# sile/libflate

Measured on AMD Instinct MI355X. Metric: gzip encode+decode throughput on 256 MiB synthetic text per GPU (uncompressed bytes through the round trip), higher is better.
Workload: dtype u8; 1 GPU; cfg2: gzip::Encoder (DefaultLz77Encoder, default options, mtime=0) + gzip::Decoder on TEXT(268435456 B) per GPU, write schedule S8K (8192-byte writes); bytes_per_gpu=268435456, schedule=S8K, compressed_bytes=129579521, parallelism=1 rank

## Files before the change

### libflate_amd/csrc/lfx_decode.cpp

```cpp
#include "../../include/lfx.h"

#include <hip/hip_runtime.h>

#include <algorithm>
#include <cstddef>
#include <cstdio>
#include <cstdlib>
#include <cstring>
#include <mutex>
#include <string>
#include <vector>

#include "lfx_decode_int.h"
#include "lfx_container.h"
#include "lfx_index.h"
#include "lfx_bgzf.h"
#include "lfx_dict.h"

static_assert(offsetof(lfx::DecStream, out_off) == 16 && sizeof(lfx::DecStream) % 8 == 0, "checksum_ranges stride");
static_assert(offsetof(lfx::InflateResult, out_len) == 8 && sizeof(lfx::InflateResult) % 8 == 0, "checksum_ranges stride");
#include "lfx_device.h"
#include "lfx_abi_guard.h"

using namespace lfx;

namespace {

int size_member(Ctx *c, const uint8_t *d_in, uint64_t n, uint64_t off0, MemberResult &mr);

int verify_trailer(Ctx *c, int format, const uint8_t *d_in, uint64_t tpos, uint64_t need, const uint8_t *d_out, const MemberResult &mr,
                   DecodeOutcome &oc) {
    hipStream_t st = c->stream;
    uint8_t t[8];
    EncodeResult er{};
    if (mr.ck_done) {
        er.crc32 = mr.crc32; er.adler32 = mr.adler32;
        memcpy(t, mr.trailer, need);
    } else {
        const uint64_t nspans = ck_nspans(mr.out_len);
        int rc;
        if ((rc = c->d_ck.reserve(12 * nspans))) return rc;
        uint32_t *ck = (uint32_t *)c->d_ck.p;
        LAUNCH_TRY(launch_checksum(st, d_out, mr.out_len, ck, ck + nspans, ck + 2 * nspans, (EncodeResult *)c->d_res.p,
                                   format == LFX_GZIP ? 1 : format == LFX_ZLIB ? 2 : 3));
        HIP_TRY(hipMemcpyAsync(c->h_res, c->d_res.p, sizeof(EncodeResult), hipMemcpyDeviceToHost, st));
        HIP_TRY(hipMemcpyAsync(t, d_in + tpos, need, hipMemcpyDeviceToHost, st));
        HIP_TRY(hipStreamSynchronize(st));
        c->phase("checksum");
        er = *(EncodeResult *)c->h_res;
    }
    if (const int bad = check_trailer(format, t, er.crc32, er.adler32, oc.msg)) oc.status = bad;
    return LFX_OK;
}

int member_loop(Ctx *c, int format, uint32_t flags, const uint8_t *d_in, uint64_t n, uint8_t *d_out, uint64_t cap, bool sizes_only,
                DecodeOutcome &oc, uint64_t base, uint64_t out_at, bool one_member, std::vector<lfx_member> *members,
                const lfx_dict *dict = nullptr) {
    (void)hipSetDevice(c->device);
    hipStream_t st = c->stream;
    bool first = base == 0;
    oc.consumed = base;
    oc.out_len = oc.delivered_len = out_at;
    int rc;
    if (!sizes_only && (rc = c->d_res.reserve(256))) return rc;
    if ((rc = c->d_small.reserve(70000))) return rc;
    for (;;) {
        uint64_t off0 = 0;
        uint64_t dict_hist = dict && format == LFX_DEFLATE ? dict->usable : 0;
        if (format != LFX_DEFLATE) {
            DecStream ds{base, n - base, 0, 0};
            DecHeader dh{};
            c->pin_reset();
            HIP_TRY(c->small_up(c->d_small.p, &ds, sizeof ds, st));
            if (dict)
                LAUNCH_TRY(launch_container_dict(st, 1, d_in, (const DecStream *)c->d_small.p,
                                                 (DecHeader *)((uint8_t *)c->d_small.p + 256), dict->id));
            else
            LAUNCH_TRY(launch_container(st, format, 1, d_in, (const DecStream *)c->d_small.p,
                                        (DecHeader *)((uint8_t *)c->d_small.p + 256)));
            HIP_TRY(c->small_down(&dh, (uint8_t *)c->d_small.p + 256, sizeof dh, st));
            HIP_TRY(c->small_sync(st));
            if (dh.status != 0) {
                if (!first && dh.status == 2) {
                    oc.consumed = n;
                    break;
                }
                oc.status = map_status(dh.status);
                oc.header_failed = first;
                oc.msg = format_error(dh.err, dh.a0, dh.a1);
                oc.consumed = base + dh.deflate_off;
                oc.out_len = oc.delivered_len = out_at;
                return LFX_OK;
            }
            off0 = dh.deflate_off;
            if (dict && (dh.flags & HDR_DICT)) dict_hist = dict->usable;
        }
        if (c->idx && !sizes_only) {
            c->idx->bit_base = base * 8;
            c->idx->out_base = out_at;
            c->idx->cand.push_back(IdxCand{(base + off0) * 8, (base + off0) * 8, out_at, IDX_BTYPE_READ});
        }
        MemberResult mr;
        if (sizes_only) rc = size_member(c, d_in + base, n - base, off0, mr);
        else {
            mr.ck_mode = ck_mode_of(format);
            mr.trailer_len = trailer_len(format);
            rc = inflate_member(c, d_in + base, n - base, off0, d_out + out_at, cap - out_at, mr, ~0ull, ~0ull, false, dict_hist,
                                dict_hist ? dict->d_win : nullptr);
        }
        if (rc) return rc;
        oc.out_len = out_at + mr.out_len;
        oc.delivered_len = out_at + mr.blk_out_start;
        oc.consumed = base + mr.end_byte;
        if (mr.status != LFX_OK) { oc.status = mr.status; oc.msg = mr.msg; return LFX_OK; }
        if (format != LFX_DEFLATE) {
            const uint64_t need = trailer_len(format);
            const uint64_t tpos = base + mr.end_byte;
            if (n - tpos < need) {
                oc.status = LFX_E_UNEXPECTED_EOF;
                oc.msg = "failed to fill whole buffer";
                oc.consumed = n;
                return LFX_OK;
            }
            oc.consumed = tpos + need;
            if (!sizes_only) {
                if ((rc = verify_trailer(c, format, d_in, tpos, need, d_out + out_at, mr, oc))) return rc;
                if (oc.status != LFX_OK) return LFX_OK;
            }
        }
        if (members) members->push_back(lfx_member{base, oc.consumed - base, out_at, mr.out_len});
        out_at = oc.out_len;
        if (one_member) { oc.more = true; break; }
        if (!(format == LFX_GZIP && (flags & LFX_DEC_MULTI))) break;
        base = oc.consumed;
        first = false;
    }
    oc.out_len = oc.delivered_len = out_at;
    return LFX_OK;
}

int decode_stream(Ctx *c, int format, uint32_t flags, const uint8_t *d_in, uint64_t n, uint8_t *d_out,
                  uint64_t cap, DecodeOutcome &oc, uint64_t base = 0, uint64_t out_at = 0, bool one_member = false,
                  std::vector<lfx_member> *members = nullptr, const lfx_dict *dict = nullptr) {
    return member_loop(c, format, flags, d_in, n, d_out, cap, false, oc, base, out_at, one_member, members, dict);
}

int parse_headers(Ctx *c, int format, const uint8_t *d_in, const std::vector<DecStream> &streams, std::vector<DecHeader> &hdrs,
                  size_t extra_bytes = 0, DecStream **d_streams = nullptr, DecHeader **d_hdrs = nullptr, const lfx_dict *dict = nullptr) {
    hipStream_t st = c->stream;
    const uint32_t count = (uint32_t)streams.size();
    const size_t sz_streams = sizeof(DecStream) * count, sz_hdr = sizeof(DecHeader) * count;
    int rc;
    if ((rc = c->d_dec_blocks.reserve(sz_streams + sz_hdr + extra_bytes))) return rc;
    DecStream *ds = (DecStream *)c->d_dec_blocks.p;
    DecHeader *dh = (DecHeader *)((uint8_t *)c->d_dec_blocks.p + sz_streams);
    HIP_TRY(hipMemcpyAsync(ds, streams.data(), sz_streams, hipMemcpyHostToDevice, st));
    if (dict && format == LFX_ZLIB) LAUNCH_TRY(launch_container_dict(st, count, d_in, ds, dh, dict->id));
    else LAUNCH_TRY(launch_container(st, format, count, d_in, ds, dh));
    hdrs.assign(count, DecHeader{});
    if (format != LFX_DEFLATE) {
        HIP_TRY(hipMemcpyAsync(hdrs.data(), dh, sz_hdr, hipMemcpyDeviceToHost, st));
// ... 1499 lines not shown
```

### libflate_amd/csrc/lfx_decode.h

```cpp
#pragma once
#include <hip/hip_runtime.h>
#include <stdint.h>

#include "lfx_common.h"
#include "lfx_blk.h"

namespace lfx {

struct DecStream {
    uint64_t in_off, in_len;
    uint64_t out_off, out_cap;
};
enum : uint32_t { JOB_SINGLE_BLOCK = 1, JOB_COUNT_ONLY = 2 };
struct InflateJob {
    uint64_t in_off;
    uint64_t in_len;
    uint64_t start_bit;
    uint64_t out_off, out_cap;
    uint64_t hist_avail;
    uint64_t stop_bit;
    uint32_t flags;
    uint32_t dict_len;
};
struct InflateResult {
// ... 27 lines not shown
int launch_blk_walk_size(hipStream_t st, const uint8_t *in, uint64_t nbytes, const WalkJob *jobs, uint32_t njobs,
                         WalkResult *results, bool small_blocks);
size_t blk_tabs_bytes();
int launch_blk_scan(hipStream_t st, const uint8_t *in, uint64_t nbytes, const BlkJob *jobs, uint32_t njobs,
                    BlkInfo *infos, BlkLanes *lanes, void *tabs = nullptr,
                    bool small_blocks = false);
int launch_blk_scan_store(hipStream_t st, const uint8_t *in, uint64_t nbytes, const BlkJob *jobs, uint32_t njobs,
                          BlkInfo *infos, BlkLanes *lanes, void *tabs, uint32_t *temp, BlkLanesX *lanesx);
int launch_blk_place(hipStream_t st, const BlkEmit *jobs, uint32_t njobs, const BlkLanes *lanes, const BlkLanesX *lanesx,
                     const uint32_t *temp, uint32_t *codes, uint32_t *flags, BlkUnits *units, uint32_t unit_target,
                     uint32_t *job_flags, uint32_t free_shift);
int launch_blk_emit(hipStream_t st, const uint8_t *in, uint64_t nbytes, const BlkEmit *jobs, uint32_t njobs,
                    const BlkLanes *lanes, uint32_t *codes, uint32_t *flags, BlkUnits *units, uint32_t unit_target,
                    uint32_t *job_flags = nullptr,
                    const void *tabs = nullptr,
                    uint32_t free_shift = 17,
                    bool large_blocks = false,
                    bool small_blocks = false);
int launch_blk_materialize(hipStream_t st, const uint8_t *in, const BlkEmit *jobs, uint32_t njobs,
                           const BlkLanes *lanes, const BlkUnits *units, const uint32_t *codes, uint8_t *out,
                           uint64_t *dbg);
int launch_blk_materialize_dict(hipStream_t st, const uint8_t *in, const BlkEmit *jobs, uint32_t njobs, const BlkUnits *units,
                                const uint32_t *codes, uint8_t *out, const uint8_t *dict_end);

int launch_blk_materialize_sym(hipStream_t st, const uint8_t *in, const BlkEmit *jobs, uint32_t njobs,
                               const BlkUnits *units, const uint32_t *codes, uint16_t *sym,
                               bool few_units = false );
int launch_window_chain(hipStream_t st, const uint16_t *sym, const SymUnit *units, uint32_t nunits, uint8_t *windows,
                        const uint8_t *init_win = nullptr);
size_t window_prefix_scratch_bytes(uint32_t nunits);
int launch_window_prefix(hipStream_t st, const uint16_t *sym, const SymUnit *units, uint32_t nunits, void *scratch,
                         uint8_t *windows, const uint8_t *init_win = nullptr);
int launch_window_rank_map(hipStream_t st, const uint16_t *sym, const SymUnit *units, uint32_t nunits, void *scratch, uint16_t *out_map);
int launch_bytes_to_map(hipStream_t st, const uint8_t *out, uint64_t len, uint16_t *map);
int launch_window_ranks(hipStream_t st, const uint16_t *maps, uint32_t nranks, uint8_t *win);
int launch_sym_substitute(hipStream_t st, const uint16_t *sym, const SymUnit *units, uint32_t nunits,
                          const uint8_t *windows, uint8_t *out, uint64_t max_len, const uint8_t *init_win = nullptr);

int launch_container(hipStream_t st, int format, uint32_t count, const uint8_t *in,
                     const DecStream *streams, DecHeader *hdrs);
int launch_inflate(hipStream_t st, const uint8_t *in, uint8_t *out, const InflateJob *jobs,
                   InflateResult *results, uint32_t njobs);
int launch_container_dict(hipStream_t st, uint32_t count, const uint8_t *in, const DecStream *streams, DecHeader *hdrs,
                          uint32_t dict_id);
int launch_inflate_dict(hipStream_t st, const uint8_t *in, uint8_t *out, const InflateJob *jobs, InflateResult *results,
                        uint32_t njobs, const uint8_t *dict_end);
constexpr uint32_t FIND_SHARDS = 256;
constexpr uint32_t FIND_HDR_WORDS = 1024, FIND_HDR_FINAL = 320, FIND_HDR_DBG = 360, FIND_HDR_READ = 512 ;
constexpr uint32_t FIND2_GROUPS = 16, FIND_HDR_WORK = 512, FIND_HDR_WORK_STRIDE = 32;
inline uint32_t find_shard_cap(uint64_t comp_bytes) {
    const uint64_t want = comp_bytes / 4000;
    return (uint32_t)(want < 4096 ? 4096 : want > (1u << 23) ? (1u << 23) : want);
}
int launch_find_stage1(hipStream_t st, const uint8_t *in, uint64_t nbytes, uint64_t first_byte,
                       uint32_t *count, uint64_t *cand, uint32_t shard_cap, uint64_t final_from_bit, uint32_t n_cu);
int launch_find_stage2(hipStream_t st, const uint8_t *in, uint64_t nbytes, const uint64_t *cand,
                       uint32_t shard_cap, const uint32_t *count ,
                       uint32_t *work ,
                       uint32_t *final_count, uint64_t *final_list, uint32_t final_cap, uint32_t n_cu,
                       uint64_t *dbg = nullptr ,
                       int exp = 0 );
constexpr uint64_t MEMBER_TILE = 16384;
constexpr uint64_t MEMBER_SKIP = ~0ull;
inline uint64_t member_tiles(uint64_t n) { return (n + MEMBER_TILE - 1) / MEMBER_TILE; }
int launch_member_count(hipStream_t st, const uint8_t *in, uint64_t n, uint32_t *tile_count );
int launch_member_emit(hipStream_t st, const uint8_t *in, uint64_t n, const uint64_t *tile_pos ,
                       uint64_t *out, uint64_t cap);
int launch_verify_trailers(hipStream_t st, int format, uint32_t count, const uint8_t *in,
                           const DecStream *streams, const DecHeader *hdrs, InflateResult *results,
                           const uint32_t *crc, const uint32_t *adler, uint64_t *consumed);
}
```

### libflate_amd/csrc/lfx_decode_int.h

```cpp
#pragma once
#include <hip/hip_runtime.h>

#include <string>
#include <vector>

#include "../../include/lfx.h"
#include "lfx_container.h"
#include "lfx_verdict.h"
#include "lfx_ctx.h"
#include "lfx_decode.h"
#include "lfx_stages.h"
#include "lfx_try.h"

namespace lfx {

struct MemberResult {
    int status = LFX_OK;
    uint64_t out_len = 0;
    uint64_t blk_out_start = 0;
    uint64_t end_byte = 0;
    std::string msg;
    uint64_t end_bit = 0;
    bool final_seen = false;
    bool need_cap = false;
    int ck_mode = 0;
    uint32_t trailer_len = 0;
    bool ck_done = false;
    uint32_t crc32 = 0, adler32 = 1;
    uint8_t trailer[8] = {0, 0, 0, 0, 0, 0, 0, 0};
};

struct DecodeOutcome {
    int status = LFX_OK;
    uint64_t out_len = 0, delivered_len = 0, consumed = 0;
    bool header_failed = false;
    bool more = false;
    std::string msg;
};

int run_jobs(Ctx *c, const uint8_t *d_in, uint8_t *d_out, const std::vector<InflateJob> &jobs, std::vector<InflateResult> &res,
             const uint8_t *dict_end = nullptr);

struct HuffProbe { uint64_t in_off, in_len; InflateResult r; };
inline bool huff_verdict(const InflateResult &r) { return r.status == 1 && r.err == ERR_HUFF; }
int huff_consumed(Ctx *c, const uint8_t *d_in, const std::vector<HuffProbe> &probes, std::vector<uint64_t> &used);

int inflate_member(Ctx *c, const uint8_t *d_in, uint64_t n, uint64_t off0, uint8_t *d_out, uint64_t cap, MemberResult &mr,
                   uint64_t start_bit0 = ~0ull, uint64_t stop_bit = ~0ull, bool partial = false, uint64_t hist = 0,
                   const uint8_t *hist_win = nullptr);


struct FindBufs {
    uint32_t shard_cap = 0, final_cap = 0;
    uint32_t *d_count = nullptr;
    uint64_t *d_final = nullptr;
    uint64_t *d_cand = nullptr;
};
struct Found {
    std::vector<uint64_t> cand;
    bool overflow = false;
    uint32_t n1 = 0;
};
int find_launch(Ctx *c, const uint8_t *d_in, uint64_t n, uint64_t off0, uint64_t final_from, FindBufs &fb);
int find_collect(Ctx *c, const uint8_t *d_in, uint64_t n, const FindBufs &fb, Found &out);
inline uint64_t find_final_from(uint64_t n, uint64_t comp) {
    const uint64_t tail_bytes = std::max<uint64_t>(comp / 8, 8ull << 20);
    return comp > tail_bytes ? (n - tail_bytes) * 8 : 0;
}

bool plan_store(Ctx *c, BlkJob *bj, uint32_t nj);

int rescan_widen(Ctx *c, const uint8_t *d_in, uint64_t n, const std::vector<uint64_t> &starts, uint32_t nc,
                 std::vector<BlkInfo> &bi, std::vector<uint32_t> &slot, std::vector<uint8_t> &stored, bool scan_small);

struct EmitBufs {
    uint32_t *d_flags = nullptr;
    BlkEmit *d_emit = nullptr;
};
int emit_codes(Ctx *c, const uint8_t *d_in, uint64_t n, const std::vector<BlkEmit> &emit, uint64_t total_codes, uint32_t n_placed,
               uint32_t free_shift, bool scan_small, EmitBufs &eb);

int scan_round(Ctx *c, const uint8_t *d_in, uint64_t n, const std::vector<BlkJob> &bj, bool want_tabs, std::vector<BlkInfo> &bi,
               bool &small, bool stamp = false);
int emit_round(Ctx *c, const uint8_t *d_in, uint64_t n, const std::vector<BlkEmit> &emit, uint64_t total_codes, bool small,
               uint8_t *d_out, std::vector<uint32_t> &jf, bool stamp = false, const uint8_t *dict_end = nullptr);

}
```

### libflate_amd/csrc/lfx_decode_kernels.hip

```cpp
#include <hip/hip_runtime.h>
#include <stdint.h>

#include "lfx_common.h"
#include "lfx_decode.h"
#include "lfx_container.h"

namespace lfx {

__device__ __forceinline__ uint32_t ld1(gptr_u8 p) { return *p; }

__global__ void container_kernel(int format, uint32_t count, const uint8_t *__restrict__ in,
                                 const DecStream *__restrict__ streams, DecHeader *__restrict__ hdrs) {
    const uint32_t i = blockIdx.x * blockDim.x + threadIdx.x;
    if (i >= count) return;
    hdrs[i] = parse_container(format, in + streams[i].in_off, streams[i].in_len, nullptr);
}
__global__ void container_dict_kernel(uint32_t count, const uint8_t *__restrict__ in, const DecStream *__restrict__ streams,
                                      DecHeader *__restrict__ hdrs, uint32_t dict_id) {
    const uint32_t i = blockIdx.x * blockDim.x + threadIdx.x;
    if (i >= count) return;
    hdrs[i] = resolve_fdict(parse_container(1, in + streams[i].in_off, streams[i].in_len, nullptr), dict_id);
}

constexpr uint32_t WIN_BYTES = 2048;
// ... 173 lines not shown
#undef LFX_INFLATE_DICT

constexpr uint32_t FIND_DWORDS = 1024;
#ifndef LFX_FIND_FLUSH
#define LFX_FIND_FLUSH 4
#endif
constexpr uint32_t FIND_FLUSH = LFX_FIND_FLUSH;
constexpr uint32_t FIND_WL = 64 * FIND_FLUSH < 256 ? 256 : 64 * FIND_FLUSH;
constexpr uint32_t FIND_LIST = 4096;
struct FindLut { uint16_t v[4096]; };
constexpr FindLut make_find_lut() {
    FindLut t{};
    for (uint32_t i = 0; i < 4096; ++i) {
        uint32_t k = 0, u = 0;
        for (int f = 0; f < 4; ++f) { const uint32_t l = (i >> (3 * f)) & 7; if (l) { k += 128u >> l; u++; } }
        t.v[i] = (uint16_t)(k | (u << 12));
    }
    return t;
}
__device__ const FindLut g_find_lut = make_find_lut();

constexpr uint32_t FIND_CLASSES = 16, FIND_SUB = FIND_SHARDS / FIND_CLASSES;
static_assert(FIND_CLASSES * FIND_SUB == FIND_SHARDS, "lists");
struct FindCls { uint8_t v[512]; };
constexpr FindCls make_find_cls() {
    constexpr uint32_t th[15] = {432, 568, 652, 832, 944, 1076, 1420, 1604, 2008, 2710, 3016, 4978, 5184, 5664, 9820};
    FindCls t{};
    for (uint32_t i = 0; i < 512; ++i) {
        const uint32_t l16 = i & 7, l17 = (i >> 3) & 7, l18 = i >> 6;
        const uint32_t p16 = l16 ? 128u >> l16 : 0u, p17 = l17 ? 128u >> l17 : 0u, p18 = l18 ? 128u >> l18 : 0u;
        const uint32_t rest = p16 + p17 + p18 <= 128 ? 128 - p16 - p17 - p18 : 0;
        const uint32_t e2 = p18 * 149 + p17 * 13 + p16 * 9 + 2 * rest;
        uint32_t c = 0;
        for (uint32_t k = 0; k < 15; ++k) c += e2 >= th[k] ? 1u : 0u;
        t.v[i] = (uint8_t)c;
    }
    return t;
}
__device__ const FindCls g_find_cls = make_find_cls();

__device__ __forceinline__ uint32_t find_wave_inclusive_sum(uint32_t x) {
    x += (uint32_t)__builtin_amdgcn_update_dpp(0, (int)x, 0x111, 0xF, 0xF, true);
    x += (uint32_t)__builtin_amdgcn_update_dpp(0, (int)x, 0x112, 0xF, 0xF, true);
    x += (uint32_t)__builtin_amdgcn_update_dpp(0, (int)x, 0x114, 0xF, 0xF, true);
    x += (uint32_t)__builtin_amdgcn_update_dpp(0, (int)x, 0x118, 0xF, 0xF, true);
    x += (uint32_t)__builtin_amdgcn_update_dpp(0, (int)x, 0x142, 0xA, 0xF, false);
    x += (uint32_t)__builtin_amdgcn_update_dpp(0, (int)x, 0x143, 0xC, 0xF, false);
    return x;
}

__global__ __launch_bounds__(256) void find_blocks_stage1(const uint8_t *__restrict__ in, uint64_t nbytes,
                                                          uint64_t first_byte, uint32_t *__restrict__ count,
                                                          uint64_t *__restrict__ cand, uint32_t shard_cap,
                                                          uint64_t final_from_bit, uint32_t ntiles) {
    __shared__ __attribute__((aligned(16))) uint32_t sd[FIND_DWORDS + 4];
    __shared__ __attribute__((aligned(16))) uint16_t lut[4096];
    __shared__ uint16_t list[FIND_LIST];
    __shared__ uint64_t wl[FIND_WL];
    __shared__ uint32_t wn, s_wtot[4], ccnt[FIND_CLASSES], cbase[FIND_CLASSES];
    if (threadIdx.x == 0) wn = 0;
    if (threadIdx.x < FIND_CLASSES) ccnt[threadIdx.x] = 0;
    const uint32_t tid = threadIdx.x, lane = tid & 63, wave = tid >> 6;
    const uint64_t a = (uint64_t)in;
    gptr_u32 w = (gptr_u32)(a & ~3ull);
    const uint64_t shift = a & 3;
    const uint64_t wlast = (shift + nbytes + 3) / 4 - 1;
    const uint64_t stream_bits = nbytes * 8, lo_bit = first_byte * 8;
    const uint32_t sub = blockIdx.x % FIND_SUB;
    {
        const uint4 *gl = (const uint4 *)g_find_lut.v;
        const uint4 l0 = gl[tid], l1 = gl[tid + 256];
        ((uint4 *)lut)[tid] = l0;
        ((uint4 *)lut)[tid + 256] = l1;
    }
    uint32_t v[5];
    auto tile_w0 = [&](uint32_t tile) { return (first_byte + (uint64_t)tile * (4 * FIND_DWORDS) + shift) >> 2; };
    auto fetch = [&](uint32_t tile) {
        const uint64_t tw0 = tile_w0(tile);
#pragma unroll
        for (uint32_t k = 0; k < 5; ++k) { const uint64_t idx = tw0 + tid + 256 * k; v[k] = w[idx < wlast ? idx : wlast]; }
    };
    uint32_t done = 0;
    if (blockIdx.x < ntiles) fetch(blockIdx.x);
    for (uint32_t tile = blockIdx.x; tile < ntiles; tile += gridDim.x) {
        const uint64_t w0 = tile_w0(tile);
        __syncthreads();
#pragma unroll
        for (uint32_t k = 0; k < 5; ++k) { const uint32_t i = tid + 256 * k; if (i < FIND_DWORDS + 4) sd[i] = v[k]; }
        __syncthreads();
        if (tile + gridDim.x < ntiles) fetch(tile + gridDim.x);
        for (uint32_t t0 = 0; t0 < FIND_DWORDS; t0 += 256) {
            const uint32_t t = t0 + tid;
            const uint32_t d0 = sd[t], d1 = sd[t + 1];
            const uint64_t dword_bit0 = (4 * (w0 + t) - shift) * 8;
            const uint32_t allow_final = dword_bit0 + 32 > final_from_bit ? ~0u : 0u;
            const uint64_t lo = (uint64_t)d0 | (uint64_t)d1 << 32;
            uint32_t pm = (uint32_t)(~(lo >> 1) & (lo >> 2)) & (~d0 | allow_final);
            const uint32_t cnt = (uint32_t)__popc(pm);
            const uint32_t incl = find_wave_inclusive_sum(cnt);
            if (lane == 63) s_wtot[wave] = incl;
            __syncthreads();
            uint32_t pos = incl - cnt, total = 0;
#pragma unroll
            for (uint32_t j = 0; j < 4; ++j) { const uint32_t wj = s_wtot[j]; pos += j < wave ? wj : 0u; total += wj; }
            while (pm) {
                const uint32_t ph = (uint32_t)__builtin_ctz(pm);
                pm &= pm - 1;
                list[pos++] = (uint16_t)(t << 5 | ph);
            }
            __syncthreads();
            for (uint32_t i = tid; i < total; i += 256) {
                const uint32_t e = list[i], te = e >> 5, ph = e & 31;
                const uint32_t e0 = sd[te], e1 = sd[te + 1], e2 = sd[te + 2], e3 = sd[te + 3];
                const uint32_t x0 = __builtin_amdgcn_alignbit(e1, e0, ph), x1 = __builtin_amdgcn_alignbit(e2, e1, ph),
                               x2 = __builtin_amdgcn_alignbit(e3, e2, ph);
                const uint32_t hlit = (x0 >> 3) & 31, hdist = (x0 >> 8) & 31, hclen = (x0 >> 13) & 15;
                if (hlit > 29 || hdist > 29) continue;
                const uint32_t nb = 3 * (hclen + 4);
                uint32_t f0 = __builtin_amdgcn_alignbit(x1, x0, 17), f1 = __builtin_amdgcn_alignbit(x2, x1, 17);
                const uint32_t m0 = nb >= 32 ? ~0u : (1u << nb) - 1u, m1 = nb > 32 ? (1u << (nb - 32)) - 1u : 0u;
                f0 &= m0;
                f1 &= m1;
                const uint32_t acc = (uint32_t)lut[f0 & 4095] + lut[(f0 >> 12) & 4095] + lut[__builtin_amdgcn_alignbit(f1, f0, 24) & 4095] +
                                     lut[(f1 >> 4) & 4095] + lut[(f1 >> 16) & 4095];
                if ((acc & 0xFFF) != 128 || (acc >> 12) < 2) continue;
                const uint64_t bit = (4 * (w0 + te) - shift) * 8 + ph;
                if ((int64_t)bit < (int64_t)lo_bit || bit + 96 > stream_bits) continue;
                const uint32_t slot = atomicAdd(&wn, 1u);
                if (slot < FIND_WL) wl[slot] = bit | (uint64_t)g_find_cls.v[f0 & 511u] << 56;
            }
        }
        const bool last = tile + gridDim.x >= ntiles;
        if (++done < FIND_FLUSH && !last) continue;
        done = 0;
        __syncthreads();
        const uint32_t mine = wn;
        if (mine > FIND_WL) {
            if (threadIdx.x == 0) atomicAdd(&count[FIND_SHARDS], 1u);
            return;
        }
        uint32_t cls[FIND_WL / 256], rnk[FIND_WL / 256];
#pragma unroll
        for (uint32_t q = 0; q < FIND_WL / 256; ++q) {
            const uint32_t k = threadIdx.x + 256 * q;
            cls[q] = k < mine ? (uint32_t)(wl[k] >> 56) : 0u;
            rnk[q] = k < mine ? atomicAdd(&ccnt[cls[q]], 1u) : 0u;
        }
        __syncthreads();
        if (threadIdx.x < FIND_CLASSES && ccnt[threadIdx.x]) cbase[threadIdx.x] = atomicAdd(&count[threadIdx.x * FIND_SUB + sub], ccnt[threadIdx.x]);
        __syncthreads();
#pragma unroll
        for (uint32_t q = 0; q < FIND_WL / 256; ++q) {
            const uint32_t k = threadIdx.x + 256 * q;
            if (k < mine) {
                const uint32_t at = cbase[cls[q]] + rnk[q];
                if (at < shard_cap) cand[(uint64_t)(cls[q] * FIND_SUB + sub) * shard_cap + at] = wl[k] & ((1ull << 56) - 1);
            }
        }
        __syncthreads();
        if (threadIdx.x == 0) wn = 0;
        if (threadIdx.x < FIND_CLASSES) ccnt[threadIdx.x] = 0;
    }
}

__global__ void verify_trailers_kernel(int format, uint32_t count, const uint8_t *__restrict__ in,
                                       const DecStream *__restrict__ streams,
                                       const DecHeader *__restrict__ hdrs,
                                       InflateResult *__restrict__ results,
                                       const uint32_t *__restrict__ crc, const uint32_t *__restrict__ adler,
                                       uint64_t *__restrict__ consumed) {
// ... 12 lines not shown
            const uint8_t *t = in + streams[i].in_off + used;
            const uint32_t need = format == 2 ? 8 : 4;
            if (n - used < need) { r.status = 2; r.err = ERR_EOF; used = n; }
            else if (format == 2) {
                const uint32_t c = (uint32_t)t[0] | (uint32_t)t[1] << 8 | (uint32_t)t[2] << 16 | (uint32_t)t[3] << 24;
                used += 8;
                if (c != crc[i]) { r.status = 1; r.err = ERR_CRC32; r.a0 = crc[i]; r.a1 = c; }
            } else {
                const uint32_t a = (uint32_t)t[0] << 24 | (uint32_t)t[1] << 16 | (uint32_t)t[2] << 8 | t[3];
                used += 4;
                if (a != adler[i]) { r.status = 1; r.err = ERR_ADLER32; r.a0 = adler[i]; r.a1 = a; }
            }
        }
    }
    results[i] = r;
    consumed[i] = used;
}

#define LFX_LAUNCH_CHECK()                          \
    do {                                            \
        hipError_t e_ = hipGetLastError();          \
        if (e_ != hipSuccess) return (int)e_;       \
    } while (0)

int launch_container(hipStream_t st, int format, uint32_t count, const uint8_t *in,
                     const DecStream *streams, DecHeader *hdrs) {
    if (!count) return 0;
    hipLaunchKernelGGL(container_kernel, dim3((count + 63) / 64), dim3(64), 0, st, format, count, in, streams, hdrs);
    LFX_LAUNCH_CHECK();
    return 0;
}
int launch_inflate(hipStream_t st, const uint8_t *in, uint8_t *out, const InflateJob *jobs,
                   InflateResult *results, uint32_t njobs) {
    if (!njobs) return 0;
    hipLaunchKernelGGL(inflate_kernel, dim3(njobs), dim3(64), 0, st, in, out, jobs, results);
    LFX_LAUNCH_CHECK();
    return 0;
}
int launch_container_dict(hipStream_t st, uint32_t count, const uint8_t *in, const DecStream *streams, DecHeader *hdrs,
                          uint32_t dict_id) {
    if (!count) return 0;
    hipLaunchKernelGGL(container_dict_kernel, dim3((count + 63) / 64), dim3(64), 0, st, count, in, streams, hdrs, dict_id);
    LFX_LAUNCH_CHECK();
    return 0;
}
int launch_inflate_dict(hipStream_t st, const uint8_t *in, uint8_t *out, const InflateJob *jobs, InflateResult *results,
                        uint32_t njobs, const uint8_t *dict_end) {
    if (!njobs) return 0;
    hipLaunchKernelGGL(inflate_dict_kernel, dim3(njobs), dim3(64), 0, st, in, out, jobs, results, dict_end);
    LFX_LAUNCH_CHECK();
    return 0;
}
int launch_find_stage1(hipStream_t st, const uint8_t *in, uint64_t nbytes, uint64_t first_byte,
                       uint32_t *count, uint64_t *cand, uint32_t shard_cap, uint64_t final_from_bit, uint32_t n_cu) {
    if (nbytes <= first_byte) return 0;
    const uint64_t n = nbytes - first_byte;
    const uint64_t ntiles = div_up(n + 4, 4 * FIND_DWORDS);
    if (ntiles > 0xFFFFFFFFull) return (int)hipErrorInvalidValue;
    static int per_cu_dev[64] = {};
    int dev_ = 0;
    (void)hipGetDevice(&dev_);
    int &per_cu = per_cu_dev[dev_ & 63];
    if (per_cu == 0) {
        int nb = 0;
        if (hipOccupancyMaxActiveBlocksPerMultiprocessor(&nb, (const void *)find_blocks_stage1, 256, 0) != hipSuccess || nb < 1) {
            (void)hipGetLastError();
            nb = 4;
        }
        per_cu = nb;
    }
    const uint64_t resident = (uint64_t)per_cu * (n_cu ? n_cu : 256u);
    hipLaunchKernelGGL(find_blocks_stage1, dim3((uint32_t)(ntiles < resident ? ntiles : resident)), dim3(256), 0, st, in, nbytes,
                       first_byte, count, cand, shard_cap, final_from_bit, (uint32_t)ntiles);
    LFX_LAUNCH_CHECK();
    return 0;
}
int launch_verify_trailers(hipStream_t st, int format, uint32_t count, const uint8_t *in,
                           const DecStream *streams, const DecHeader *hdrs, InflateResult *results,
                           const uint32_t *crc, const uint32_t *adler, uint64_t *consumed) {
    if (!count) return 0;
    hipLaunchKernelGGL(verify_trailers_kernel, dim3((count + 63) / 64), dim3(64), 0, st, format, count, in,
                       streams, hdrs, results, crc, adler, consumed);
    LFX_LAUNCH_CHECK();
    return 0;
}
}
```

### libflate_amd/csrc/lfx_member.cpp

```cpp
#include "lfx_decode_int.h"

#include <algorithm>
#include <cstdio>
#include <cstring>

#include "lfx_index.h"

namespace lfx {

int run_jobs(Ctx *c, const uint8_t *d_in, uint8_t *d_out, const std::vector<InflateJob> &jobs,
             std::vector<InflateResult> &res, const uint8_t *dict_end) {
    const size_t n = jobs.size();
    res.resize(n);
    if (!n) return LFX_OK;
    int rc;
    if ((rc = c->d_dec_streams.reserve(sizeof(InflateJob) * n))) return rc;
    if ((rc = c->d_dec_state.reserve(sizeof(InflateResult) * n))) return rc;
    HIP_TRY(hipMemcpyAsync(c->d_dec_streams.p, jobs.data(), sizeof(InflateJob) * n, hipMemcpyHostToDevice, c->stream));
    if (dict_end)
        LAUNCH_TRY(launch_inflate_dict(c->stream, d_in, d_out, (const InflateJob *)c->d_dec_streams.p,
                                       (InflateResult *)c->d_dec_state.p, (uint32_t)n, dict_end));
    else
        LAUNCH_TRY(launch_inflate(c->stream, d_in, d_out, (const InflateJob *)c->d_dec_streams.p,
                                  (InflateResult *)c->d_dec_state.p, (uint32_t)n));
    HIP_TRY(hipMemcpyAsync(res.data(), c->d_dec_state.p, sizeof(InflateResult) * n, hipMemcpyDeviceToHost, c->stream));
    HIP_TRY(hipStreamSynchronize(c->stream));
    return LFX_OK;
}


int find_launch(Ctx *c, const uint8_t *d_in, uint64_t n, uint64_t off0, uint64_t final_from, FindBufs &fb) {
    hipStream_t st = c->stream;
    const uint64_t comp = n - off0;
    fb.shard_cap = find_shard_cap(comp);
    fb.final_cap = (uint32_t)std::min<uint64_t>(std::max<uint64_t>(1u << 16, comp / 4096), 1u << 24);
    int rc;
    if ((rc = c->d_dec_cand.reserve(8ull * fb.shard_cap * FIND_SHARDS + 8ull * fb.final_cap + 4 * FIND_HDR_WORDS))) return rc;
    fb.d_count = (uint32_t *)c->d_dec_cand.p;
    fb.d_final = (uint64_t *)((uint8_t *)c->d_dec_cand.p + 4 * FIND_HDR_WORDS);
    fb.d_cand = fb.d_final + fb.final_cap;
    HIP_TRY(hipMemsetAsync(fb.d_count, 0, 4 * FIND_HDR_WORDS, st));
    LAUNCH_TRY(launch_find_stage1(st, d_in, n, off0, fb.d_count, fb.d_cand, fb.shard_cap, final_from, (uint32_t)std::max(c->n_cu, 1)));
    return LFX_OK;
}

int find_collect(Ctx *c, const uint8_t *d_in, uint64_t n, const FindBufs &fb, Found &out) {
    hipStream_t st = c->stream;
    uint32_t *d_count = fb.d_count, *d_final_count = d_count + FIND_HDR_FINAL;
    const uint32_t n_cu = (uint32_t)std::max(c->n_cu, 1);
    const int find2_exp = c->diag.find2_exp >= 1 && c->diag.find2_exp <= 4 ? c->diag.find2_exp : 0;
    if (find2_exp) {
        LAUNCH_TRY(launch_find_stage2(st, d_in, n, fb.d_cand, fb.shard_cap, d_count, d_count + FIND_HDR_WORK, d_final_count, fb.d_final,
                                      fb.final_cap, n_cu, nullptr, find2_exp));
        HIP_TRY(hipMemsetAsync(d_count + FIND_HDR_FINAL, 0, 4, st));
        HIP_TRY(hipMemsetAsync(d_count + FIND_HDR_WORK, 0, 4 * (FIND_HDR_WORDS - FIND_HDR_WORK), st));
        c->phase("find2x");
    }
    LAUNCH_TRY(launch_find_stage2(st, d_in, n, fb.d_cand, fb.shard_cap, d_count, d_count + FIND_HDR_WORK, d_final_count, fb.d_final,
                                  fb.final_cap, n_cu, c->diag.debug ? (uint64_t *)(d_count + FIND_HDR_DBG) : nullptr));
    constexpr uint32_t HEAD_N = 1024;
    const uint32_t head_n = std::min<uint32_t>(HEAD_N, fb.final_cap);
    std::vector<uint64_t> back(FIND_HDR_WORDS / 2 + head_n);
    HIP_TRY(c->small_down(back.data(), d_count, 8ull * back.size(), st));
    HIP_TRY(c->small_sync(st));
    const uint32_t *hc = (const uint32_t *)back.data();
    out.overflow = hc[FIND_SHARDS] != 0;
    out.n1 = 0;
    for (uint32_t k = 0; k < FIND_SHARDS; k++) { if (hc[k] > fb.shard_cap) out.overflow = true; out.n1 += hc[k]; }
    if (c->diag.debug) {
        uint64_t d[7];
        memcpy(d, hc + FIND_HDR_DBG, sizeof d);
        fprintf(stderr, "[lfx] finder stage 2: batches=%llu cycles per batch: stage+fields=%llu table=%llu walk=%llu; steps per batch=%.1f "
                "restagings=%llu; wavefront lives (sum)=%llu\n", (unsigned long long)d[5], (unsigned long long)(d[0] / (d[5] ? d[5] : 1)),
                (unsigned long long)(d[1] / (d[5] ? d[5] : 1)), (unsigned long long)(d[2] / (d[5] ? d[5] : 1)),
                (double)d[3] / (double)(d[5] ? d[5] : 1), (unsigned long long)d[4], (unsigned long long)d[6]);
    }
    out.cand.clear();
    if (out.overflow) return LFX_OK;
    const uint32_t nf = std::min(hc[FIND_HDR_FINAL], fb.final_cap);
    out.cand.assign(back.begin() + FIND_HDR_WORDS / 2, back.begin() + FIND_HDR_WORDS / 2 + std::min(nf, head_n));
    out.cand.resize(nf);
    if (nf > head_n) HIP_TRY(hipMemcpy(out.cand.data() + head_n, fb.d_final + head_n, 8ull * (nf - head_n), hipMemcpyDeviceToHost));
    return LFX_OK;
}

bool plan_store(Ctx *c, BlkJob *bj, uint32_t nj) {
    const uint64_t off = plan_store_regions(bj, nj, c->diag.store_tight);
    if (off * 4 > (16ull << 30) || c->d_dec_temp.reserve(off * 4) || c->d_dec_lanesx.reserve(sizeof(BlkLanesX) * (size_t)(nj + 1))) {
        clear_store_regions(bj, nj);
        return false;
    }
    return true;
}

int rescan_widen(Ctx *c, const uint8_t *d_in, uint64_t n, const std::vector<uint64_t> &starts, uint32_t nc,
                 std::vector<BlkInfo> &bi, std::vector<uint32_t> &slot, std::vector<uint8_t> &stored, bool scan_small) {
    hipStream_t st = c->stream;
    const size_t tab_bytes = blk_tabs_bytes();
    auto start_at = [&](size_t i) { return i < starts.size() ? starts[i] : n * 8; };
    for (uint32_t widen = 2; widen <= 6; widen++) {
        std::vector<uint32_t> redo;
        for (uint32_t i = 0; i < nc; i++) if (bi[slot[i]].status == BLK_NO_EOB && i + widen <= starts.size()) redo.push_back(i);
        if (redo.empty()) break;
        std::vector<BlkJob> rj(redo.size());
        for (size_t q = 0; q < redo.size(); q++) rj[q] = BlkJob{starts[redo[q]], start_at(redo[q] + widen)};
        int rc;
        if ((rc = c->d_dec_tmp.reserve(sizeof(BlkJob) * redo.size()))) return rc;
        BlkJob *d_rj = (BlkJob *)c->d_dec_tmp.p;
        HIP_TRY(hipMemcpyAsync(d_rj, rj.data(), sizeof(BlkJob) * redo.size(), hipMemcpyHostToDevice, st));
        for (size_t q = 0; q < redo.size(); q++) {
            slot[redo[q]] = redo[q];
            stored[redo[q]] = 0;
            LAUNCH_TRY(launch_blk_scan(st, d_in, n, d_rj + q, 1, (BlkInfo *)c->d_dec_state.p + redo[q],
                                       (BlkLanes *)c->d_dec_blocks.p + redo[q],
                                       (uint8_t *)c->d_dec_tabs.p + tab_bytes * redo[q], scan_small));
        }
        for (size_t q = 0; q < redo.size(); q++)
            HIP_TRY(hipMemcpyAsync(&bi[redo[q]], (BlkInfo *)c->d_dec_state.p + redo[q], sizeof(BlkInfo), hipMemcpyDeviceToHost, st));
        HIP_TRY(hipStreamSynchronize(st));
    }
    return LFX_OK;
}

int emit_codes(Ctx *c, const uint8_t *d_in, uint64_t n, const std::vector<BlkEmit> &emit, uint64_t total_codes, uint32_t n_placed,
               uint32_t free_shift, bool scan_small, EmitBufs &eb) {
    hipStream_t st = c->stream;
    const uint32_t ne = (uint32_t)emit.size();
    int rc;
    if ((rc = c->d_dec_tmp.reserve(sizeof(BlkEmit) * (size_t)ne + 64))) return rc;
    if ((rc = c->d_hist.reserve(sizeof(BlkUnits) * (size_t)ne + 64))) return rc;
    if ((rc = c->d_codes.reserve(4 * std::max<uint64_t>(total_codes, 1)))) return rc;
    eb.d_flags = (uint32_t *)c->d_dec_tmp.p;
    eb.d_emit = (BlkEmit *)((uint8_t *)c->d_dec_tmp.p + 64);
    {
        std::vector<uint8_t> upl(64 + sizeof(BlkEmit) * (size_t)ne, 0);
// ... 58 lines not shown
    else
        LAUNCH_TRY(launch_blk_materialize(st, d_in, d_emit, ne, (const BlkLanes *)c->d_dec_cand.p, (const BlkUnits *)c->d_hist.p,
                                          (const uint32_t *)c->d_codes.p, d_out, nullptr));
    if (stamp) c->phase("lz77_copy");
    jf.resize(ne);
    HIP_TRY(hipMemcpyAsync(jf.data(), d_jf, 4ull * ne, hipMemcpyDeviceToHost, st));
    HIP_TRY(hipStreamSynchronize(st));
    return LFX_OK;
}


namespace {

struct Member {
    Ctx *c;
    const uint8_t *d_in;
    uint64_t n, off0;
    uint8_t *d_out;
    uint64_t cap;
    uint64_t first_bit, stop_bit;
    bool partial;
    uint64_t hist;
    const uint8_t *hist_win;
    uint64_t comp;
    uint64_t end_bits() const { return n * 8; }
};

struct Chain {
    std::vector<BlkEmit> emit;
    uint64_t pos;
    uint64_t total = 0, total_codes = 0;
    uint64_t last_end = 0;
    bool ok = false, final = false;
    bool front_bad = false;
    bool pieces = false;
    bool pieces_multi = false;
    bool units_per_piece = false;
    bool scan_small = false;
    uint32_t n_placed = 0;
    uint32_t n_on_demand = 0;
    explicit Chain(uint64_t first_bit) : pos(first_bit) {}
    BlkEmit &push(const BlkInfo &r, uint32_t slot, uint64_t hist) {
        emit.push_back(blk_emit_of(r, pos, slot, total, total_codes, hist + total));
        total += r.n_out;
        total_codes += r.n_codes;
        return emit.back();
    }
    void close_block(const BlkInfo &r) {
        last_end = r.end_bit;
        if (r.bfinal) { ok = true; final = true; } else pos = r.end_bit;
    }
};

int find_starts(const Member &m, std::vector<uint64_t> &starts, Found &fd) {
    Ctx *c = m.c;
    FindBufs fb;
    int rc;
    const uint64_t final_from = c->diag.no_final_cand ? ~0ull >> 1 : find_final_from(m.n, m.comp);
    if ((rc = find_launch(c, m.d_in, m.n, m.off0, final_from, fb))) return rc;
    c->phase("find1");
    if ((rc = find_collect(c, m.d_in, m.n, fb, fd))) return rc;
    starts.clear();
    starts.push_back(m.first_bit);
    if (fd.overflow) return LFX_OK;
    c->phase("find2");
    for (uint64_t b : fd.cand) if (b != m.first_bit) starts.push_back(b);
    std::sort(starts.begin(), starts.end());
    return LFX_OK;
}

int scan_pieces(const Member &m, const std::vector<BlkJob> &jobs, uint32_t slot0, std::vector<BlkInfo> &infos) {
    Ctx *c = m.c;
    hipStream_t st = c->stream;
    const uint32_t nj = (uint32_t)jobs.size();
    infos.resize(nj);
    HIP_TRY(hipMemcpyAsync((BlkJob *)c->d_dec_streams.p + slot0, jobs.data(), sizeof(BlkJob) * nj, hipMemcpyHostToDevice, st));
    LAUNCH_TRY(launch_blk_scan(st, m.d_in, m.n, (const BlkJob *)c->d_dec_streams.p + slot0, nj, (BlkInfo *)c->d_dec_state.p + slot0,
                               (BlkLanes *)c->d_dec_blocks.p + slot0, (uint8_t *)c->d_dec_tabs.p + blk_tabs_bytes() * slot0));
    HIP_TRY(hipMemcpyAsync(infos.data(), (BlkInfo *)c->d_dec_state.p + slot0, sizeof(BlkInfo) * nj, hipMemcpyDeviceToHost, st));
    HIP_TRY(hipStreamSynchronize(st));
    return LFX_OK;
}
int reserve_scan_slots(Ctx *c, size_t nslots) {
    int rc;
    if ((rc = c->d_dec_streams.reserve(sizeof(BlkJob) * nslots))) return rc;
    if ((rc = c->d_dec_state.reserve(sizeof(BlkInfo) * nslots))) return rc;
    if ((rc = c->d_dec_blocks.reserve(sizeof(BlkLanes) * nslots))) return rc;
    return c->d_dec_tabs.reserve(blk_tabs_bytes() * nslots);
}

int pieces_over_ranges(const Member &m, const std::vector<uint64_t> &starts, Chain &ch) {
    Ctx *c = m.c;
    const uint32_t nc = (uint32_t)starts.size();
    const uint64_t end_bits = m.end_bits();
    auto start_at = [&](uint32_t i) { return i < nc ? starts[i] : end_bits; };
    const uint64_t ptarget = (uint64_t)std::max<int64_t>(2ll * std::max(c->n_cu, 1) - (int64_t)nc, (int64_t)nc);
    const uint64_t PIECE_BITS = piece_bits(end_bits - m.first_bit, ptarget), OVERLAP = piece_overlap(PIECE_BITS);
    std::vector<BlkJob> pj;
    std::vector<uint32_t> first_piece(nc + 1, 0);
    for (uint32_t i = 0; i < nc; i++) {
        first_piece[i] = (uint32_t)pj.size();
        add_pieces(pj, starts[i], start_at(i + 1), PIECE_BITS, OVERLAP);
    }
    first_piece[nc] = (uint32_t)pj.size();
    const uint32_t npj = (uint32_t)pj.size();
    ch.units_per_piece = npj >= (uint32_t)std::max(c->n_cu, 1);
    constexpr uint32_t REPAIRS = 2;
    const uint32_t repair_slots = REPAIRS * (2 * (uint32_t)((end_bits - m.first_bit) / nc / PIECE_BITS + 2) + 4);
    const uint32_t nslots = npj + repair_slots;
    int rc;
    if ((rc = reserve_scan_slots(c, nslots))) return rc;
    std::vector<BlkInfo> pi;
    if ((rc = scan_pieces(m, pj, 0, pi))) return rc;
    bool fail = false;
    auto walk_range = [&](const BlkInfo *infos, uint32_t cnt, uint32_t slot0) -> int {
        uint64_t prev_end = 0;
        for (uint32_t q = 0; q < cnt; q++) {
            const BlkInfo &r = infos[q];
            if (r.status == BLK_BAD || r.btype == 0 || (q && r.data_bit != prev_end) || r.end_bit <= ch.pos || r.end_bit > end_bits) return 2;
            ch.push(r, slot0 + q, m.hist);
// ... 292 lines not shown
    mr.out_len = total;
    mr.blk_out_start = total;
    mr.end_byte = end_byte;
    mr.end_bit = end_bit;
    mr.final_seen = ch.final;
    done = true;
    return LFX_OK;
}

int serial_walk(const Member &m, MemberResult &mr) {
    Ctx *c = m.c;
    const uint64_t n = m.n;
    InflateJob j{};
    j.in_off = 0; j.in_len = n; j.start_bit = m.first_bit;
    j.out_off = 0; j.out_cap = m.cap; j.hist_avail = m.hist; j.flags = 0;
    j.dict_len = m.hist_win ? (uint32_t)m.hist : 0;
    j.stop_bit = m.stop_bit == ~0ull ? 0 : m.stop_bit;
    std::vector<InflateResult> res;
    int rc;
    if ((rc = run_jobs(c, m.d_in, m.d_out, {j}, res, m.hist_win ? m.hist_win + MAX_WINDOW : nullptr))) return rc;
    c->phase("serial");
    InflateResult &r = res[0];
    uint64_t huff_used = ~0ull;
    if (huff_verdict(r) && m.stop_bit == ~0ull && !m.partial && (m.hist == 0 || m.hist_win)) {
        std::vector<uint64_t> used;
        if ((rc = huff_consumed(c, m.d_in, {HuffProbe{0, n, r}}, used))) return rc;
        huff_used = used[0];
    }
    if (m.stop_bit != ~0ull && r.status == 0 && (r.final_seen || r.end_bit != m.stop_bit)) {
        r.status = 1; r.err = ERR_HUFF; r.a0 = r.a1 = 0;
    }
    mr.status = map_status(r.status);
    mr.out_len = r.out_len;
    mr.blk_out_start = r.status ? r.blk_out_start : r.out_len;
    mr.end_byte = huff_used != ~0ull ? huff_used : std::min<uint64_t>((r.end_bit + 7) / 8, n);
    mr.end_bit = r.end_bit;
    mr.final_seen = r.status == 0 && r.final_seen;
    mr.msg = format_error(r.err, r.a0, r.a1);
    if (m.partial && r.status != 0 && (r.status == 2 || r.status == 3 || r.end_bit + 64 >= n * 8)) {
        mr.status = LFX_OK;
        mr.out_len = mr.blk_out_start = r.blk_out_start;
        mr.end_bit = r.blk_start_bit;
        mr.end_byte = r.blk_start_bit / 8;
        mr.final_seen = false;
        mr.need_cap = r.status == 3 && r.blk_out_start == 0;
        mr.msg.clear();
    }
    return LFX_OK;
}

}

int inflate_member(Ctx *c, const uint8_t *d_in, uint64_t n, uint64_t off0, uint8_t *d_out, uint64_t cap, MemberResult &mr,
                   uint64_t start_bit0, uint64_t stop_bit, bool partial, uint64_t hist, const uint8_t *hist_win) {
    const Member m{c, d_in, n, off0, d_out, cap, start_bit0 == ~0ull ? off0 * 8 : start_bit0, stop_bit, partial, hist, hist ? hist_win : nullptr,
                   n > off0 ? n - off0 : 0};
    mr.end_bit = m.first_bit;
    c->pin_reset();
    bool done = false;
    if (m.comp >= (4u << 10)) {
        int rc;
        std::vector<uint64_t> starts;
        Found fd;
        const bool may_piece = stop_bit == ~0ull && !partial && !c->diag.no_pieces;
        const bool small_first = m.comp < (1536u << 10) && may_piece;
        if (small_first) starts.push_back(m.first_bit);
        else if ((rc = find_starts(m, starts, fd))) return rc;
        if (!fd.overflow) {
            Chain ch(m.first_bit);
            const uint32_t nc = (uint32_t)starts.size();
            const bool giant_blocks = nc <= 8 && m.comp / nc >= (2u << 20);
            if (may_piece && !small_first && !giant_blocks && nc >= 2 && nc <= PIECE_RANGES_MAX && m.comp / nc >= (128u << 10) &&
                (rc = pieces_over_ranges(m, starts, ch)))
                return rc;
            if (!ch.pieces && may_piece && (small_first || giant_blocks) && (rc = pieces_block_walk(m, small_first, starts, fd, ch))) return rc;
            if (!ch.pieces && !fd.overflow && (rc = block_scan(m, starts, fd.n1, ch, mr))) return rc;
            if (c->diag.debug) fprintf(stderr, "[lfx]  chain ok=%d blocks=%zu pos=%llu total=%llu on_demand=%u\n", (int)ch.ok, ch.emit.size(), (unsigned long long)ch.pos, (unsigned long long)ch.total, ch.n_on_demand);
            if (partial && ch.emit.empty() && !ch.front_bad) {
                mr.status = LFX_OK; mr.out_len = 0; mr.blk_out_start = 0; mr.final_seen = false;
                mr.end_bit = m.first_bit; mr.end_byte = m.first_bit / 8;
                return LFX_OK;
            }
            if (ch.ok && ch.total <= cap && (rc = emit_and_materialise(m, ch, mr, done))) return rc;
        }
    }
    if (done) return LFX_OK;
    if (c->diag.no_serial) { c->set_error("serial fallback disabled (LFX_NO_SERIAL)"); return LFX_E_UNSUPPORTED; }
    return serial_walk(m, mr);
}

}
```

Measured before the change: 60.19 GB/s.

## Launch block-finder alongside header parse to skip a host round trip

```diff
diff --git a/libflate_amd/csrc/lfx_decode.cpp b/libflate_amd/csrc/lfx_decode.cpp
--- a/libflate_amd/csrc/lfx_decode.cpp
+++ b/libflate_amd/csrc/lfx_decode.cpp
@@ -67,19 +67,27 @@
     for (;;) {
         uint64_t off0 = 0;
         uint64_t dict_hist = dict && format == LFX_DEFLATE ? dict->usable : 0;
+        const bool front = !sizes_only && !one_member && !members && !dict && !c->idx && find_front_ok(c, n - base);
+        Found front_fd;
         if (format != LFX_DEFLATE) {
             DecStream ds{base, n - base, 0, 0};
             DecHeader dh{};
+            DecHeader *d_dh = (DecHeader *)((uint8_t *)c->d_small.p + 256);
             c->pin_reset();
+            FindBufs front_fb;
+            if (front && (rc = find_reserve(c, n - base, front_fb))) return rc;
             HIP_TRY(c->small_up(c->d_small.p, &ds, sizeof ds, st));
             if (dict)
-                LAUNCH_TRY(launch_container_dict(st, 1, d_in, (const DecStream *)c->d_small.p,
-                                                 (DecHeader *)((uint8_t *)c->d_small.p + 256), dict->id));
+                LAUNCH_TRY(launch_container_dict(st, 1, d_in, (const DecStream *)c->d_small.p, d_dh, dict->id));
             else
-            LAUNCH_TRY(launch_container(st, format, 1, d_in, (const DecStream *)c->d_small.p,
-                                        (DecHeader *)((uint8_t *)c->d_small.p + 256)));
-            HIP_TRY(c->small_down(&dh, (uint8_t *)c->d_small.p + 256, sizeof dh, st));
-            HIP_TRY(c->small_sync(st));
+            LAUNCH_TRY(launch_container(st, format, 1, d_in, (const DecStream *)c->d_small.p, d_dh));
+            if (front) {
+                c->phase("headers");
+                if ((rc = find_front(c, d_in + base, n - base, front_fb, d_dh, dh, front_fd))) return rc;
+            } else {
+                HIP_TRY(c->small_down(&dh, d_dh, sizeof dh, st));
+                HIP_TRY(c->small_sync(st));
+            }
             if (dh.status != 0) {
                 if (!first && dh.status == 2) {
                     oc.consumed = n;
@@ -106,7 +114,7 @@
             mr.ck_mode = ck_mode_of(format);
             mr.trailer_len = trailer_len(format);
             rc = inflate_member(c, d_in + base, n - base, off0, d_out + out_at, cap - out_at, mr, ~0ull, ~0ull, false, dict_hist,
-                                dict_hist ? dict->d_win : nullptr);
+                                dict_hist ? dict->d_win : nullptr, front && format != LFX_DEFLATE ? &front_fd : nullptr);
         }
         if (rc) return rc;
         oc.out_len = out_at + mr.out_len;
diff --git a/libflate_amd/csrc/lfx_decode.h b/libflate_amd/csrc/lfx_decode.h
--- a/libflate_amd/csrc/lfx_decode.h
+++ b/libflate_amd/csrc/lfx_decode.h
@@ -103,8 +103,13 @@
     const uint64_t want = comp_bytes / 4000;
     return (uint32_t)(want < 4096 ? 4096 : want > (1u << 23) ? (1u << 23) : want);
 }
+LFX_HD inline uint64_t find_final_from(uint64_t n, uint64_t comp) {
+    const uint64_t tail_bytes = comp / 8 > (8ull << 20) ? comp / 8 : 8ull << 20;
+    return comp > tail_bytes ? (n - tail_bytes) * 8 : 0;
+}
 int launch_find_stage1(hipStream_t st, const uint8_t *in, uint64_t nbytes, uint64_t first_byte,
-                       uint32_t *count, uint64_t *cand, uint32_t shard_cap, uint64_t final_from_bit, uint32_t n_cu);
+                       uint32_t *count, uint64_t *cand, uint32_t shard_cap, uint64_t final_from_bit, uint32_t n_cu,
+                       const DecHeader *hdr = nullptr);
 int launch_find_stage2(hipStream_t st, const uint8_t *in, uint64_t nbytes, const uint64_t *cand,
                        uint32_t shard_cap, const uint32_t *count ,
                        uint32_t *work ,
diff --git a/libflate_amd/csrc/lfx_decode_int.h b/libflate_amd/csrc/lfx_decode_int.h
--- a/libflate_amd/csrc/lfx_decode_int.h
+++ b/libflate_amd/csrc/lfx_decode_int.h
@@ -45,9 +45,11 @@
 inline bool huff_verdict(const InflateResult &r) { return r.status == 1 && r.err == ERR_HUFF; }
 int huff_consumed(Ctx *c, const uint8_t *d_in, const std::vector<HuffProbe> &probes, std::vector<uint64_t> &used);
 
+struct Found;
 int inflate_member(Ctx *c, const uint8_t *d_in, uint64_t n, uint64_t off0, uint8_t *d_out, uint64_t cap, MemberResult &mr,
                    uint64_t start_bit0 = ~0ull, uint64_t stop_bit = ~0ull, bool partial = false, uint64_t hist = 0,
-                   const uint8_t *hist_win = nullptr);
+                   const uint8_t *hist_win = nullptr, const Found *front = nullptr);
+constexpr uint64_t FINDER_FIRST_BYTES = 1536ull << 10;
 
 
 struct FindBufs {
@@ -61,12 +63,12 @@
     bool overflow = false;
     uint32_t n1 = 0;
 };
+int find_reserve(Ctx *c, uint64_t comp, FindBufs &fb);
 int find_launch(Ctx *c, const uint8_t *d_in, uint64_t n, uint64_t off0, uint64_t final_from, FindBufs &fb);
-int find_collect(Ctx *c, const uint8_t *d_in, uint64_t n, const FindBufs &fb, Found &out);
-inline uint64_t find_final_from(uint64_t n, uint64_t comp) {
-    const uint64_t tail_bytes = std::max<uint64_t>(comp / 8, 8ull << 20);
-    return comp > tail_bytes ? (n - tail_bytes) * 8 : 0;
-}
+int find_collect(Ctx *c, const uint8_t *d_in, uint64_t n, const FindBufs &fb, Found &out, const DecHeader *d_hdr = nullptr,
+                 DecHeader *hdr_out = nullptr);
+bool find_front_ok(const Ctx *c, uint64_t n);
+int find_front(Ctx *c, const uint8_t *d_in, uint64_t n, const FindBufs &fb, const DecHeader *d_hdr, DecHeader &dh, Found &fd);
 
 bool plan_store(Ctx *c, BlkJob *bj, uint32_t nj);
 
diff --git a/libflate_amd/csrc/lfx_decode_kernels.hip b/libflate_amd/csrc/lfx_decode_kernels.hip
--- a/libflate_amd/csrc/lfx_decode_kernels.hip
+++ b/libflate_amd/csrc/lfx_decode_kernels.hip
@@ -249,7 +249,14 @@
 __global__ __launch_bounds__(256) void find_blocks_stage1(const uint8_t *__restrict__ in, uint64_t nbytes,
                                                           uint64_t first_byte, uint32_t *__restrict__ count,
                                                           uint64_t *__restrict__ cand, uint32_t shard_cap,
-                                                          uint64_t final_from_bit, uint32_t ntiles) {
+                                                          uint64_t final_from_bit, uint32_t ntiles,
+                                                          const DecHeader *__restrict__ hdr) {
+    uint64_t lo_byte = first_byte;
+    if (hdr) {
+        if (hdr->status != 0) return;
+        lo_byte = hdr->deflate_off;
+        final_from_bit = find_final_from(nbytes, nbytes > lo_byte ? nbytes - lo_byte : 0);
+    }
     __shared__ __attribute__((aligned(16))) uint32_t sd[FIND_DWORDS + 4];
     __shared__ __attribute__((aligned(16))) uint16_t lut[4096];
     __shared__ uint16_t list[FIND_LIST];
@@ -262,7 +269,7 @@
     gptr_u32 w = (gptr_u32)(a & ~3ull);
     const uint64_t shift = a & 3;
     const uint64_t wlast = (shift + nbytes + 3) / 4 - 1;
-    const uint64_t stream_bits = nbytes * 8, lo_bit = first_byte * 8;
+    const uint64_t stream_bits = nbytes * 8, lo_bit = lo_byte * 8;
     const uint32_t sub = blockIdx.x % FIND_SUB;
     {
         const uint4 *gl = (const uint4 *)g_find_lut.v;
@@ -292,7 +299,8 @@
             const uint64_t dword_bit0 = (4 * (w0 + t) - shift) * 8;
             const uint32_t allow_final = dword_bit0 + 32 > final_from_bit ? ~0u : 0u;
             const uint64_t lo = (uint64_t)d0 | (uint64_t)d1 << 32;
-            uint32_t pm = (uint32_t)(~(lo >> 1) & (lo >> 2)) & (~d0 | allow_final);
+            const uint64_t run2 = lo & (lo >> 1), run4 = run2 & (run2 >> 2);
+            uint32_t pm = (uint32_t)(~(lo >> 1) & (lo >> 2)) & (~d0 | allow_final) & ~(uint32_t)((run4 >> 4) | (run4 >> 9));
             const uint32_t cnt = (uint32_t)__popc(pm);
             const uint32_t incl = find_wave_inclusive_sum(cnt);
             if (lane == 63) s_wtot[wave] = incl;
@@ -311,8 +319,7 @@
                 const uint32_t e0 = sd[te], e1 = sd[te + 1], e2 = sd[te + 2], e3 = sd[te + 3];
                 const uint32_t x0 = __builtin_amdgcn_alignbit(e1, e0, ph), x1 = __builtin_amdgcn_alignbit(e2, e1, ph),
                                x2 = __builtin_amdgcn_alignbit(e3, e2, ph);
-                const uint32_t hlit = (x0 >> 3) & 31, hdist = (x0 >> 8) & 31, hclen = (x0 >> 13) & 15;
-                if (hlit > 29 || hdist > 29) continue;
+                const uint32_t hclen = (x0 >> 13) & 15;
                 const uint32_t nb = 3 * (hclen + 4);
                 uint32_t f0 = __builtin_amdgcn_alignbit(x1, x0, 17), f1 = __builtin_amdgcn_alignbit(x2, x1, 17);
                 const uint32_t m0 = nb >= 32 ? ~0u : (1u << nb) - 1u, m1 = nb > 32 ? (1u << (nb - 32)) - 1u : 0u;
@@ -431,7 +438,8 @@
     return 0;
 }
 int launch_find_stage1(hipStream_t st, const uint8_t *in, uint64_t nbytes, uint64_t first_byte,
-                       uint32_t *count, uint64_t *cand, uint32_t shard_cap, uint64_t final_from_bit, uint32_t n_cu) {
+                       uint32_t *count, uint64_t *cand, uint32_t shard_cap, uint64_t final_from_bit, uint32_t n_cu,
+                       const DecHeader *hdr) {
     if (nbytes <= first_byte) return 0;
     const uint64_t n = nbytes - first_byte;
     const uint64_t ntiles = div_up(n + 4, 4 * FIND_DWORDS);
@@ -450,7 +458,7 @@
     }
     const uint64_t resident = (uint64_t)per_cu * (n_cu ? n_cu : 256u);
     hipLaunchKernelGGL(find_blocks_stage1, dim3((uint32_t)(ntiles < resident ? ntiles : resident)), dim3(256), 0, st, in, nbytes,
-                       first_byte, count, cand, shard_cap, final_from_bit, (uint32_t)ntiles);
+                       first_byte, count, cand, shard_cap, final_from_bit, (uint32_t)ntiles, hdr);
     LFX_LAUNCH_CHECK();
     return 0;
 }
diff --git a/libflate_amd/csrc/lfx_member.cpp b/libflate_amd/csrc/lfx_member.cpp
--- a/libflate_amd/csrc/lfx_member.cpp
+++ b/libflate_amd/csrc/lfx_member.cpp
@@ -29,9 +29,8 @@
 }
 
 
-int find_launch(Ctx *c, const uint8_t *d_in, uint64_t n, uint64_t off0, uint64_t final_from, FindBufs &fb) {
-    hipStream_t st = c->stream;
-    const uint64_t comp = n - off0;
+int find_reserve(Ctx *c, uint64_t comp, FindBufs &fb) {
+    hipStream_t st = c->stream;
     fb.shard_cap = find_shard_cap(comp);
     fb.final_cap = (uint32_t)std::min<uint64_t>(std::max<uint64_t>(1u << 16, comp / 4096), 1u << 24);
     int rc;
@@ -40,11 +39,16 @@
     fb.d_final = (uint64_t *)((uint8_t *)c->d_dec_cand.p + 4 * FIND_HDR_WORDS);
     fb.d_cand = fb.d_final + fb.final_cap;
     HIP_TRY(hipMemsetAsync(fb.d_count, 0, 4 * FIND_HDR_WORDS, st));
-    LAUNCH_TRY(launch_find_stage1(st, d_in, n, off0, fb.d_count, fb.d_cand, fb.shard_cap, final_from, (uint32_t)std::max(c->n_cu, 1)));
-    return LFX_OK;
-}
-
-int find_collect(Ctx *c, const uint8_t *d_in, uint64_t n, const FindBufs &fb, Found &out) {
+    return LFX_OK;
+}
+int find_launch(Ctx *c, const uint8_t *d_in, uint64_t n, uint64_t off0, uint64_t final_from, FindBufs &fb) {
+    int rc;
+    if ((rc = find_reserve(c, n - off0, fb))) return rc;
+    LAUNCH_TRY(launch_find_stage1(c->stream, d_in, n, off0, fb.d_count, fb.d_cand, fb.shard_cap, final_from, (uint32_t)std::max(c->n_cu, 1)));
+    return LFX_OK;
+}
+
+int find_collect(Ctx *c, const uint8_t *d_in, uint64_t n, const FindBufs &fb, Found &out, const DecHeader *d_hdr, DecHeader *hdr_out) {
     hipStream_t st = c->stream;
     uint32_t *d_count = fb.d_count, *d_final_count = d_count + FIND_HDR_FINAL;
     const uint32_t n_cu = (uint32_t)std::max(c->n_cu, 1);
@@ -62,6 +66,7 @@
     const uint32_t head_n = std::min<uint32_t>(HEAD_N, fb.final_cap);
     std::vector<uint64_t> back(FIND_HDR_WORDS / 2 + head_n);
     HIP_TRY(c->small_down(back.data(), d_count, 8ull * back.size(), st));
+    if (d_hdr) HIP_TRY(c->small_down(hdr_out, d_hdr, sizeof *hdr_out, st));
     HIP_TRY(c->small_sync(st));
     const uint32_t *hc = (const uint32_t *)back.data();
     out.overflow = hc[FIND_SHARDS] != 0;
@@ -81,6 +86,19 @@
     out.cand.assign(back.begin() + FIND_HDR_WORDS / 2, back.begin() + FIND_HDR_WORDS / 2 + std::min(nf, head_n));
     out.cand.resize(nf);
     if (nf > head_n) HIP_TRY(hipMemcpy(out.cand.data() + head_n, fb.d_final + head_n, 8ull * (nf - head_n), hipMemcpyDeviceToHost));
+    return LFX_OK;
+}
+
+bool find_front_ok(const Ctx *c, uint64_t n) {
+    const Diag &d = c->diag;
+    return n >= FINDER_FIRST_BYTES && !d.debug && !d.no_pieces && !d.no_final_cand && !d.find2_exp;
+}
+int find_front(Ctx *c, const uint8_t *d_in, uint64_t n, const FindBufs &fb, const DecHeader *d_hdr, DecHeader &dh, Found &fd) {
+    int rc;
+    LAUNCH_TRY(launch_find_stage1(c->stream, d_in, n, 0, fb.d_count, fb.d_cand, fb.shard_cap, 0, (uint32_t)std::max(c->n_cu, 1), d_hdr));
+    c->phase("find1");
+    if ((rc = find_collect(c, d_in, n, fb, fd, d_hdr, &dh))) return rc;
+    if (dh.status != 0) fd = Found{};
     return LFX_OK;
 }
 
@@ -245,6 +263,14 @@
     }
 };
 
+void starts_of(const Member &m, const Found &fd, std::vector<uint64_t> &starts) {
+    starts.clear();
+    starts.push_back(m.first_bit);
+    if (fd.overflow) return;
+    m.c->phase("find2");
+    for (uint64_t b : fd.cand) if (b != m.first_bit) starts.push_back(b);
+    std::sort(starts.begin(), starts.end());
+}
 int find_starts(const Member &m, std::vector<uint64_t> &starts, Found &fd) {
     Ctx *c = m.c;
     FindBufs fb;
@@ -253,12 +279,7 @@
     if ((rc = find_launch(c, m.d_in, m.n, m.off0, final_from, fb))) return rc;
     c->phase("find1");
     if ((rc = find_collect(c, m.d_in, m.n, fb, fd))) return rc;
-    starts.clear();
-    starts.push_back(m.first_bit);
-    if (fd.overflow) return LFX_OK;
-    c->phase("find2");
-    for (uint64_t b : fd.cand) if (b != m.first_bit) starts.push_back(b);
-    std::sort(starts.begin(), starts.end());
+    starts_of(m, fd, starts);
     return LFX_OK;
 }
 
@@ -657,7 +678,7 @@
 }
 
 int inflate_member(Ctx *c, const uint8_t *d_in, uint64_t n, uint64_t off0, uint8_t *d_out, uint64_t cap, MemberResult &mr,
-                   uint64_t start_bit0, uint64_t stop_bit, bool partial, uint64_t hist, const uint8_t *hist_win) {
+                   uint64_t start_bit0, uint64_t stop_bit, bool partial, uint64_t hist, const uint8_t *hist_win, const Found *front) {
     const Member m{c, d_in, n, off0, d_out, cap, start_bit0 == ~0ull ? off0 * 8 : start_bit0, stop_bit, partial, hist, hist ? hist_win : nullptr,
                    n > off0 ? n - off0 : 0};
     mr.end_bit = m.first_bit;
@@ -668,8 +689,9 @@
         std::vector<uint64_t> starts;
         Found fd;
         const bool may_piece = stop_bit == ~0ull && !partial && !c->diag.no_pieces;
-        const bool small_first = m.comp < (1536u << 10) && may_piece;
+        const bool small_first = m.comp < FINDER_FIRST_BYTES && may_piece;
         if (small_first) starts.push_back(m.first_bit);
+        else if (front) { fd = *front; starts_of(m, fd, starts); }
         else if ((rc = find_starts(m, starts, fd))) return rc;
         if (!fd.overflow) {
             Chain ch(m.first_bit);
```

New measurement: 60.21 GB/s, median of 3. No clear change (+0.0%).
